# codebydant/sfM_danPipeline

Hardware: AMD Instinct MI355X
Metric: image-pairs matched/sec + BA iterations/sec (200 cams, 100k pts, 1M obs) (higher is better)
Workload: dtype i8

## Files before the change

sfm_danpipeline_amd/csrc/ba.hip:

```cpp
#include "common.h"
#include "ba_front_plan.h"
#include "ba_setup.h"
#include <algorithm>
#include <atomic>
#include <chrono>
#include <cmath>
#include <condition_variable>
#include <cstring>
#include <mutex>
#include <functional>
#include <map>
#include <thread>
#include <vector>
#include <float.h>
#include <unistd.h>

namespace {

constexpr int CAMD = 40;
using bsetup::SC;
constexpr int RED2_SLOTS = 32, RED2_SUM_N = 8 + 4 * RED2_SLOTS, RED2_TMP = RED2_SUM_N, RED2_INFO = RED2_SUM_N + 1,
              RED2_N = RED2_SUM_N + 8;
constexpr int RED2_TIMEOUT = 4;
constexpr int INFO_FINISHER_TIMEOUT = -2;
using bsetup::Chunk;

struct BaDev {
  int nc, np, no, dim, ld;
  const int* optr;
  const int* ocam;
  const double2* oxy;
  double* cams;
  double* pts;
  double* focal;
  double* camd;
  double* cams_c;
  double* pts_c;
  double* focal_c;
  double* camd_c;
  double* scale_c;
  double* scale_p;
  double* iscale_p;
  double* scale_f;
  double* diag;
  double* red;
  double* z;
  double* xinv;
  double* red2;
  int* info;
  struct LmDev* lm;
  double* step_part;
  int step_total;
  int cam_parts;
  int decide_here;
  int rank;
  int step_last;
  double* lm_host;
// ... 395 lines not shown
      asm volatile("s_memtime %0\n\ts_memrealtime %1\n\ts_waitcnt lgkmcnt(0)" : "=s"(t_), "=s"(r_)::"memory"); \
      g_elim_wg[5 * blockIdx.x + slot] = t_;                                                         \
      g_elim_wg[5 * blockIdx.x + 2 + slot] = r_;                                                     \
      if (slot == 0) {                                                                               \
        unsigned id_, xcc_;                                                                          \
        asm volatile("s_getreg_b32 %0, hwreg(HW_REG_HW_ID)\n\ts_getreg_b32 %1, hwreg(HW_REG_XCC_ID)" : "=s"(id_), "=s"(xcc_)); \
        g_elim_wg[5 * blockIdx.x + 4] = ((unsigned long long)xcc_ << 32) | id_;                      \
      }                                                                                              \
    }                                                                                                \
  } while (0)
#define EL_STAMP(slot, cond)                                                         \
  do {                                                                               \
    unsigned long long t_;                                                           \
    asm volatile("s_memtime %0\n\ts_waitcnt lgkmcnt(0)" : "=s"(t_)::"memory");       \
    ((blockIdx.x == 0 && wave == 0 && (cond)) ? g_elim_stamps : g_elim_dump)[slot] = t_; \
  } while (0)
#define EL_STAMPW(slot)                                                        \
  do {                                                                         \
    unsigned long long t_;                                                     \
    asm volatile("s_memtime %0\n\ts_waitcnt lgkmcnt(0)" : "=s"(t_)::"memory"); \
    ((blockIdx.x == 0) ? g_elim_stamps : g_elim_dump)[slot] = t_;              \
  } while (0)
#else
#define EL_STAMP(slot, cond)
#define EL_STAMPW(slot)
#define EL_WG(slot)
#endif
using bsetup::ELIM_SLAB_FF;
using bsetup::ELIM_SLAB;
using bsetup::FP;
constexpr int MP = 80;

typedef __attribute__((address_space(3))) double lds_double;
struct CamLds {
  const lds_double* base;
  const lds_double* dbase;
  __device__ __forceinline__ double operator[](int e) const { return e < 12 ? base[e * 16] : dbase[e * 16]; }
};

#ifndef SFM_ELIM_LB
#define SFM_ELIM_LB __launch_bounds__(512)
#endif
struct ElimShape {
  static constexpr int LP = 10;
  static constexpr int PPW = 64 / LP;
  static constexpr int KST = (3 * PPW + 3) / 4;
  static constexpr int PROWS = 4 * KST;
};
__device__ __forceinline__ void group10_sum12(double (&red)[12], double* R, int lane, int q, int o) {
  constexpr int PR = 66;
  typedef __attribute__((address_space(3))) double ldsd;
  ldsd* Rl = (ldsd*)R;
#pragma unroll
  for (int v = 0; v < 12; ++v) Rl[v * PR + lane] = red[v];
  __builtin_amdgcn_fence(__ATOMIC_RELEASE, "wavefront");
  __builtin_amdgcn_wave_barrier();
  __builtin_amdgcn_fence(__ATOMIC_ACQUIRE, "wavefront");
  const int qq = q < 6 ? q : 5;
  const ldsd* a = Rl + o * PR + qq * 10;
  const ldsd* b = Rl + (10 + (o & 1)) * PR + qq * 10;
  double s0 = a[0], s1 = b[0];
#pragma unroll
  for (int j = 1; j < 10; ++j) {
    s0 += a[j];
    s1 += b[j];
  }
// ... 333 lines not shown
  for (int idx = tid; idx < 36 * FP; idx += (int)blockDim.x) {
    const int e = idx / FP, slot = idx - e * FP;
    if (slot >= n) continue;
    double v = 0.0;
    for (int w = 0; w < nw; ++w) v += s_F[(w * 36 + e) * FP + slot];
    s_F[e * FP + slot] = v;
    if (norms || e >= 33) continue;
    if (e < 21) {
      int i = 0, rem = e;
      while (rem >= 6 - i) {
        rem -= 6 - i;
        ++i;
      }
      g_sub(6 * slot + i, 6 * slot + i + rem, v);
    } else if (e < 27) {
      g_sub(6 * slot + e - 21, 6 * n, v);
    } else {
      g_sub(6 * slot + e - 27, 6 * n + 1, v);
    }
  }
  __syncthreads();
  EL_STAMP(4, true);
  if (tid < 3) {
    double v = 0.0;
    for (int slot = 0; slot < n; ++slot) v += s_F[(33 + tid) * FP + slot];
    s_F[(nw * 36 + tid) * FP] = v;
    if (!norms && tid < 2) g_sub(6 * n, 6 * n + tid, v);
  }
  __syncthreads();
  EL_STAMP(5, true);
  if (slab) {
    double* my = slab + (size_t)chunk_index * ELIM_SLAB;
    if (!norms)
      for (int k = tid; k < NT * 256; k += (int)blockDim.x) my[k] = s_G[k];
    for (int idx = tid; idx < 36 * FP; idx += (int)blockDim.x) my[ELIM_SLAB_FF + idx] = s_F[idx];
    if (tid < 3) my[ELIM_SLAB_FF + 36 * FP + tid] = s_F[(nw * 36 + tid) * FP];
    if (tid == 0) {
      double gm = 0.0, nf = 0.0;
      for (int w = 0; w < nw; ++w) {
        gm = fmax(gm, s_wv[2 * w]);
        nf += s_wv[2 * w + 1];
      }
      my[ELIM_SLAB_FF + 36 * FP + 3] = gm;
      my[ELIM_SLAB_FF + 36 * FP + 4] = nf;
      my[ELIM_SLAB_FF + 36 * FP + 5] = norms ? 0.0 : s_G[g_slot(6 * n, 6 * n)];
      my[ELIM_SLAB_FF + 36 * FP + 6] = norms ? 0.0 : s_G[g_slot(6 * n, 6 * n + 1)];
    }
    EL_STAMP(6, true);
    EL_WG(1);
#ifdef SFM_ELIM_WG_RECORDS
    if (tid == 0 && blockIdx.x < 2048) g_elim_wg[5 * blockIdx.x + 4] |= (unsigned long long)ch.cnt << 48;
#endif
    return;
  }
  double* scv = red_sc(d);
  if (lane == 0 && !norms) {
    if (nfail) atomic_add_f64(scv + 2, (double)nfail);
    atomic_max_pos_f64(scv + SC + rank, gmax);
  }
  for (int idx = tid; idx < 33 * FP; idx += (int)blockDim.x) {
    const int e = idx / FP, slot = idx - e * FP;
    if (slot >= n) continue;
    const int r0 = 6 * cams[slot];
    if (e < 21) {
      int i = 0, rem = e;
      while (rem >= 6 - i) {
        rem -= 6 - i;
        ++i;
      }
      if (rem == 0) atomic_add_f64(red_dc(d) + r0 + i, s_F[e * FP + slot]);
    } else if (e >= 27 && !norms) {
      atomic_add_f64(red_gF(d) + r0 + e - 27, s_F[e * FP + slot]);
    }
  }
  if (tid < 3) {
    const double v = s_F[(nw * 36 + tid) * FP];
    if (tid == 0) atomic_add_f64(red_dc(d) + fo, v);
    else if (norms) {
    } else if (tid == 1) atomic_add_f64(red_gF(d) + fo, v);
// ... 34 lines not shown
    double radius;
    lm_view(d, radius);
    inv_radius = 1.0 / radius;
  }
  elim_chunk<NB>(d, chunks, chunk_ids[blockIdx.x], sig_cams, inv_radius, lm_lo, lm_hi, rank, norms, slab);
}

__global__ __launch_bounds__(256) void ba_gather_slabs(const double* __restrict__ slab, const int* __restrict__ ptr,
                                                       const unsigned* __restrict__ src, const int* __restrict__ dest, int nd,
                                                       double* __restrict__ red, long long gmax_off, const LmDev* __restrict__ lm) {
  if (lm && lm->stop != LM_RUNNING) return;
  const int i = (blockIdx.x * blockDim.x + threadIdx.x) >> 4, j = threadIdx.x & 15;
  const bool live = i < nd;
  const int d = live ? dest[i] : 0;
  const int k0 = live ? ptr[i] : 0, k1 = live ? ptr[i + 1] : 0;
  if (live && d < 0) {
    double v = 0.0;
    for (int k = k0 + j; k < k1; k += 16) v = fmax(v, slab[src[k]]);
#pragma unroll
    for (int off = 8; off > 0; off >>= 1) v = fmax(v, __shfl_xor(v, off, 16));
    if (j == 0) red[gmax_off] = fmax(red[gmax_off], v);
    return;
  }
  double v = 0.0;
  for (int k = k0 + j; k < k1; k += 16) {
    const unsigned sk = src[k];
    const double x = slab[sk & 0x7fffffffu];
    v += (sk >> 31) ? -x : x;
  }
  v = row16_sum(v);
  if (live && j == 0) red[d] += v;
}

__global__ __launch_bounds__(256) void ba_gather_rows(const double* __restrict__ slab,
                                                      const int* __restrict__ colmap, const int4* __restrict__ row_hdr,
                                                      const int4* __restrict__ row_head, const int4* __restrict__ row_src, int nrows,
                                                      int row_wgs, int ld, int accw, int fo, int nchunks, const int* __restrict__ ptr,
                                                      const unsigned* __restrict__ src, const int* __restrict__ dest, int nd,
                                                      double* __restrict__ red, long long gmax_off, int rmw, const LmDev* __restrict__ lm) {
  extern __shared__ double s_acc[];
  if (lm && lm->stop != LM_RUNNING) return;
  if ((int)blockIdx.x == (int)gridDim.x - 1) {
    const int T = blockDim.x, t = threadIdx.x;
    double p[7] = {0, 0, 0, 0, 0, 0, 0};
    for (int c0 = t; c0 < nchunks; c0 += 4 * T) {
      double x[4][7];
#pragma unroll
      for (int u = 0; u < 4; ++u) {
        const double* tail = slab + (size_t)(c0 + u * T < nchunks ? c0 + u * T : c0) * ELIM_SLAB + ELIM_SLAB_FF + 36 * FP;
        x[u][0] = tail[5];
        x[u][1] = tail[6];
#pragma unroll
        for (int q = 0; q < 5; ++q) x[u][2 + q] = tail[q];
      }
      asm volatile("" ::: "memory");
#pragma unroll
      for (int u = 0; u < 4; ++u)
        if (c0 + u * T < nchunks) {
#pragma unroll
          for (int q = 0; q < 7; ++q) p[q] = q == 5 ? fmax(p[q], x[u][q]) : p[q] + x[u][q];
        }
    }
    for (int q = 0; q < 7; ++q) s_acc[q * T + t] = p[q];
    __syncthreads();
    for (int h = T >> 1; h > 0; h >>= 1) {
      if (t < h)
        for (int q = 0; q < 7; ++q) s_acc[q * T + t] = q == 5 ? fmax(s_acc[q * T + t], s_acc[q * T + t + h]) : s_acc[q * T + t] + s_acc[q * T + t + h];
      __syncthreads();
    }
    if (t < 7) {
      const size_t ssz = (size_t)ld * ld;
      const size_t at[7] = {(size_t)fo * ld + fo, ssz + fo, ssz + 2 * (size_t)ld + fo, ssz + (size_t)ld + fo, ssz + 3 * (size_t)ld,
                            (size_t)gmax_off, ssz + 3 * (size_t)ld + 2};
      const double v = s_acc[t * T], o = red[at[t]];
      red[at[t]] = t < 2 ? o - v : t == 5 ? fmax(o, v) : o + v;
    }
    return;
  }
  if ((int)blockIdx.x >= row_wgs) {
    const int i = (((int)blockIdx.x - row_wgs) * blockDim.x + threadIdx.x) >> 4, j = threadIdx.x & 15;
    const bool live = i < nd;
    const int d = live ? dest[i] : 0;
    const int k0 = live ? ptr[i] : 0, k1 = live ? ptr[i + 1] : 0;
    if (live && d < 0) {
      double v = 0.0;
      for (int k = k0 + j; k < k1; k += 16) v = fmax(v, slab[src[k]]);
#pragma unroll
      for (int off = 8; off > 0; off >>= 1) v = fmax(v, __shfl_xor(v, off, 16));
      if (j == 0) red[gmax_off] = fmax(red[gmax_off], v);
      return;
    }
    double v = 0.0;
    for (int k = k0 + j; k < k1; k += 64) {
      unsigned sk[4];
#pragma unroll
      for (int u = 0; u < 4; ++u) sk[u] = k + 16 * u < k1 ? src[k + 16 * u] : 0u;
      double x[4];
#pragma unroll
      for (int u = 0; u < 4; ++u) x[u] = slab[sk[u] & 0x7fffffffu];
#pragma unroll
      for (int u = 0; u < 4; ++u)
        if (k + 16 * u < k1) v += (sk[u] >> 31) ? -x[u] : x[u];
    }
    v = row16_sum(v);
    if (live && j == 0) red[d] += v;
    return;
  }
  const int wave = threadIdx.x >> 6, lane = threadIdx.x & 63, nw = blockDim.x >> 6;
  const int w = blockIdx.x * nw + wave;
  if (w >= nrows) return;
  double* acc = s_acc + (size_t)wave * accw;
  const int4 hdr = row_hdr[w];
  int4 my = lane < 32 ? row_head[(size_t)w * 32 + lane] : make_int4(0, 0, 0, 0);
  const int* const clist = colmap + hdr.w;
  const int nT = 6 * clist[-1], nacc = nT + 4;
  for (int c = lane; c < accw; c += 64) acc[c] = 0.0;
  const int gr = hdr.x, nsrc = hdr.y;
  const int lane_off = (lane >> 4) * 256 + (lane & 15);
  for (int kb = 0; kb < nsrc; kb += 32) {
    constexpr int GB = 32;
    const int m = nsrc - kb < 32 ? nsrc - kb : 32;
    if (kb > 0) my = lane < m ? row_src[hdr.z + (kb - 32) + lane] : make_int4(0, 0, 0, 0);
    for (int u0 = 0; u0 < m; u0 += GB) {
      double v[GB];
      int col[GB];
      bool ok[GB];
#pragma unroll
      for (int u = 0; u < GB; ++u) {
        const int uu = u0 + u < m ? u0 + u : m - 1;
        const int base = __builtin_amdgcn_readlane(my.x, uu), rec = __builtin_amdgcn_readlane(my.y, uu);
        const int cm = __builtin_amdgcn_readlane(my.z, uu), ff = __builtin_amdgcn_readlane(my.w, uu);
        const int lr = rec & 255, n = (rec >> 8) & 255, roff = (int)((unsigned)rec >> 16);
        ok[u] = u0 + u < m && ((lane >= lr && lane < 6 * n + 2) || lane >= 62);
        const int idx = lane >= 62 ? ELIM_SLAB_FF + (lane == 62 ? (ff & 0xFFFF) : (int)((unsigned)ff >> 16)) : roff + lane_off;
        v[u] = slab[(size_t)(unsigned)base + (ok[u] ? idx : 0)];
        col[u] = colmap[cm + lane];
      }
      asm volatile("" ::: "memory");
#pragma unroll
      for (int u = 0; u < GB; ++u)
        if (ok[u]) __hip_atomic_fetch_add((lds_double*)acc + col[u], v[u], __ATOMIC_RELAXED, __HIP_MEMORY_SCOPE_WORKGROUP);
    }
  }
  double* Srow = red + (size_t)gr * ld;
  const size_t ssz = (size_t)ld * ld;
  for (int c = lane; c < nacc; c += 64) {
    const double a = acc[c];
    if (a != 0.0) {
      double* at = c < nT       ? Srow + 6 * clist[c / 6] + c % 6
                   : c == nT     ? Srow + fo
                   : c == nT + 1 ? red + ssz + gr
                   : c == nT + 2 ? red + ssz + 2 * (size_t)ld + gr
                                 : red + ssz + (size_t)ld + gr;
      const double o = rmw ? *at : 0.0;
      *at = c <= nT + 1 ? o - a : o + a;
    }
  }
}

__global__ __launch_bounds__(256) void ba_cam_blocks(BaDev d, const int* __restrict__ cptr,
                                                     const int* __restrict__ cpt,
                                                     const double2* __restrict__ cxy, int nsplit,
                                                     int norms_only ,
                                                     const int2* __restrict__ cslot ,
                                                     const double* __restrict__ T, const double* __restrict__ tfu,
                                                     const double* __restrict__ pp_part, int n_part, int rank,
                                                     double* __restrict__ cb_part ,
                                                     int* __restrict__ cb_cnt ) {
  __shared__ double sh[4][36];
  __shared__ double sh2[4][33];
  __shared__ int s_last;
  {
    double radius_unused;
    lm_view(d, radius_unused);
  }
  double q[33];
#pragma unroll
  for (int e = 0; e < 33; ++e) q[e] = 0.0;
  const int c = blockIdx.x / nsplit, part = blockIdx.x - c * nsplit;
  const int k0 = cptr[c], k1 = cptr[c + 1];
  const int len = k1 - k0;
  const int per = (len + nsplit - 1) / nsplit;
  const int kb = k0 + part * per, ke = min(k1, kb + per);
  double a[36];
#pragma unroll
  for (int e = 0; e < 36; ++e) a[e] = 0.0;
  const double* cd = d.camd + (size_t)CAMD * c;
  const double* scp = norms_only ? nullptr : d.scale_c + 6 * c;
  const double sf = norms_only ? 1.0 : *d.scale_f, focal = *d.focal;
  for (int k = kb + threadIdx.x; k < ke; k += 256) {
// ... 705 lines not shown
        for (int ks = 0; ks < 16; ks += 2) {
          CHOL_MFMA(acc[0], -Lb[0][ks], Lb[0][ks]);
          CHOL_MFMA(acc[1], -Lb[0][ks], Lb[1][ks]);
          CHOL_MFMA(p0, -Lb[0][ks + 1], Lb[0][ks + 1]);
          CHOL_MFMA(p1, -Lb[0][ks + 1], Lb[1][ks + 1]);
        }
        acc[0] += p0;
        acc[1] += p1;
      }
      C2_STAMP(23);
      const double* const y0 = sYb + j16 * CBP + q;
      const double* const y1 = y0 + 16 * CBP;
      int seen = 0;
#pragma unroll 1
      for (int b = 0; b < 8; ++b) {
        if (seen <= b) seen = __builtin_amdgcn_readfirstlane(lds_wait_ge(&s_flag[F_YPROG], b + 1));
        const double Y0 = y0[4 * b], Y1 = y1[4 * b];
        CHOL_MFMA(acc[0], -Y0, Y0);
        CHOL_MFMA(acc[1], -Y0, Y1);
      }
      __builtin_amdgcn_s_setprio(3);
      C2_STAMP(3);
    } else {
      lds_wait_ge(&s_flag[F_CNT_DAA], 3);
      acc[0] = chol2_get(sDa, 0, lane);
      acc[1] = chol2_get(sDa, 2, lane);
      acc[2] = chol2_get(sDa, 3, lane);
    }
    bool bad = false;
    const int c0 = pass ? b0 : a0;
    chol2_potrf_blocks(acc, sAll + opaque(pass * 3 * T), sdi_all + opaque(pass * CB), s_flag + opaque(F_PROG_A + pass),
                       bad, lane, nullptr, ld, pass ? &s_flag[F_DBB_HI] : nullptr);
    C2_STAMP(pass ? 4 : 2);
    if (owner && bad && lane == 0) atomicExch(info, c0 + 1);
    if (!pass) {
      __builtin_amdgcn_s_setprio(1);
      if (pend) {
        double Lb[16];
#pragma unroll
        for (int ks = 0; ks < 16; ++ks) Lb[ks] = opab[32 + 16 + 4 * ks * C2_PAB];
        chol2_fold_regs(t1, Lb, Lb);
      }
      lds_wait_ge(&s_flag[F_YPROG], 8);
      const double* const yh = sYb + (16 + j16) * CBP + q;
      v4d p0 = {0.0, 0.0, 0.0, 0.0}, p1 = p0, p2 = p0;
#pragma unroll
      for (int b = 0; b < 8; b += 4) {
        const double Ya = yh[4 * b], Yb = yh[4 * b + 4], Yc = yh[4 * b + 8], Yd = yh[4 * b + 12];
        CHOL_MFMA(t1, -Ya, Ya);
        CHOL_MFMA(p0, -Yb, Yb);
        CHOL_MFMA(p1, -Yc, Yc);
        CHOL_MFMA(p2, -Yd, Yd);
      }
      t1 += (p0 + p1) + p2;
      chol2_put(sAll + 3 * T, 3, lane, t1);
      lds_flag_add(&s_flag[F_DBB_HI], lane);
      C2_STAMP(14);
    }
    if (!pass && !owner) {
      if (pend) {
        double Lb[16], Lr[2][16];
#pragma unroll
        for (int ks = 0; ks < 16; ++ks) {
          Lb[ks] = opab[32 + 16 + 4 * ks * C2_PAB];
          Lr[0][ks] = oprw[4 * ks * C2_PRW];
          Lr[1][ks] = oprw[16 + 4 * ks * C2_PRW];
        }
// ... 1100 lines not shown

struct sfmhip_ba {
  sfmhip_ctx* ctx = nullptr;
  LmState lm;
  LmDev* d_lm = nullptr;
  LmDev* h_ring = nullptr;
  LmDev* h_ring_dev = nullptr;
  unsigned lm_seq = 0;
  double* d_step_part = nullptr;
  size_t step_part_n = 0;
  bool tree_by_level = false;
  int spin_timeouts = 0;
  int nc = 0, np_in = 0, no_in = 0;
  int np = 0, no = 0;
  int dim = 0, ld = 0;
  size_t ssz = 0;
  BaDev d{};
  bool use_arena = false;
  size_t arena_off = 0, arena_need = 0;
  bool pinned_shared = false;
  std::vector<int> perm;
  std::vector<int> obs_src;
  std::vector<int> cxy_src;
  double2* d_oxy_w = nullptr;
  int* d_obs_src = nullptr;
  std::vector<unsigned char> h_cam_used;
  unsigned char* d_cam_used = nullptr;
  bool cam_used_known = false;
  double* d_flag = nullptr;
  bool chol_attr_set = false;
  Chunk* d_chunks = nullptr;
  bool elim_deterministic = !(getenv("SFMHIP_BA_DETERMINISTIC") && atoi(getenv("SFMHIP_BA_DETERMINISTIC")) == 0);
  double* d_slab = nullptr;
  int* d_gth_ptr[2] = {nullptr, nullptr};
  unsigned* d_gth_src[2] = {nullptr, nullptr};
  int* d_gth_dest[2] = {nullptr, nullptr};
  int n_gth[2] = {0, 0};
  int4* d_grow_hdr = nullptr;
  int4* d_grow_head = nullptr;
  int4* d_grow_src = nullptr;
  int* d_grow_colmap = nullptr;
  int n_grow = 0, grow_waves = 4, grow_accw = 64, n_chunks = 0;
  int* d_chunk_ids[8] = {nullptr, nullptr, nullptr, nullptr, nullptr, nullptr, nullptr, nullptr};
  int n_chunk_ids[8] = {0, 0, 0, 0, 0, 0, 0, 0};
  int* d_sig_cams = nullptr;
  int* d_cptr = nullptr;
  int* d_cpt = nullptr;
  double2* d_cxy = nullptr;
  int cam_split = 1;
  int dense_xb = 0;
  double* d_back_part = nullptr;
  double* d_cb_part = nullptr;
  int* d_cb_cnt = nullptr;
  int* d_fb_points = nullptr;
  int* d_pp_obase = nullptr;
  int n_fb = 0;
  int2* d_cslot = nullptr;
  double* d_ppT = nullptr;
  double* d_tfu = nullptr;
  double* d_pp_part = nullptr;
  int n_pp_part = 0;
  int* d_pair_ptr = nullptr;
  int2* d_pair_cams = nullptr;
  int2* d_pair_ent = nullptr;
  int n_pairs_pp = 0;
  long long tree_dbg_ints = 0, tree_dbg_doubles = 0;
// ... 249 lines not shown
  double2* d_oxy = nullptr;
  b->red_count = b->ssz + 3 * (size_t)b->ld + SC + 64 + RED2_N + b->ssz;
#define BA_A(ptr, n)                         \
  if (rc == SFMHIP_OK) rc = ba_alloc(b, &(ptr), (size_t)(n))
  BA_A(d_optr, b->np + 1);
  BA_A(d_ocam, b->no);
  BA_A(d_oxy, b->no);
  BA_A(b->d_obs_src, b->no);
  BA_A(d.cams, 6 * n_cam);
  BA_A(d.pts, 3 * (size_t)b->np);
  BA_A(d.focal, 1);
  BA_A(d.camd, (size_t)CAMD * n_cam);
  BA_A(d.cams_c, 6 * n_cam);
  BA_A(d.pts_c, 3 * (size_t)b->np);
  BA_A(d.focal_c, 1);
  BA_A(d.camd_c, (size_t)CAMD * n_cam);
  BA_A(d.scale_c, 6 * n_cam);
  BA_A(d.scale_p, 3 * (size_t)b->np);
  BA_A(d.iscale_p, 3 * (size_t)b->np);
  BA_A(d.scale_f, 1);
  BA_A(d.diag, b->ld);
  BA_A(d.red, b->red_count);
  BA_A(d.z, b->ld);
  if (rc == SFMHIP_OK) {
    d.red2 = d.red + b->ssz + 3 * (size_t)b->ld + SC + 64;
    d.info = (int*)(d.red2 + RED2_INFO);
    d.xinv = d.red2 + RED2_N;
  }
  BA_A(b->d_cam_used, n_cam);
  BA_A(b->d_flag, 2);
  BA_A(b->d_chunks, S.chunks.size());
  if (!S.gth_dest[0].empty() || !S.gth_dest[1].empty() || !S.grow_hdr.empty()) {
    BA_A(b->d_slab, S.chunks.size() * (size_t)ELIM_SLAB);
    for (int m = 0; m < 2; ++m) {
      BA_A(b->d_gth_ptr[m], S.gth_ptr[m].size());
      BA_A(b->d_gth_src[m], S.gth_src[m].size());
      BA_A(b->d_gth_dest[m], S.gth_dest[m].size());
    }
    if (!S.grow_hdr.empty()) {
      BA_A(b->d_grow_hdr, S.grow_hdr.size());
      BA_A(b->d_grow_head, S.grow_head.size());
      BA_A(b->d_grow_src, S.grow_over.size());
      BA_A(b->d_grow_colmap, S.grow_colmap.size());
    }
  }
  for (int c = 0; c < 8; ++c) BA_A(b->d_chunk_ids[c], S.ids[c].size());
  BA_A(b->d_sig_cams, S.sig_cams.size());
  BA_A(b->d_cptr, S.cptr.size());
  BA_A(b->d_cpt, S.cpt.size());
  BA_A(b->d_cxy, S.cpt.size());
  BA_A(b->d_fb_points, S.fb.size());
  BA_A(b->d_pp_obase, S.pp_obase.size());
  BA_A(b->d_cslot, S.cslot.size());
  BA_A(b->d_ppT, 18 * S.cslot.size());
  BA_A(b->d_tfu, 6 * S.fb.size());
  b->n_pp_part = (int)((S.fb.size() * PP_LANES + 255) / 256);
  BA_A(b->d_pp_part, 8 * (size_t)b->n_pp_part);
  if (b->cam_split > 1) {
    BA_A(b->d_cb_part, 66 * (size_t)n_cam * b->cam_split);
    BA_A(b->d_cb_cnt, n_cam);
    if (rc == SFMHIP_OK && hipMemset(b->d_cb_cnt, 0, sizeof(int) * (size_t)n_cam) != hipSuccess) rc = SFMHIP_ERR_HIP;
  }
  {
    const int nt = b->ld / CB;
    b->dense_xb = nt >= DENSE_XB_MIN_NT ? DENSE_XB : 0;
    if (b->dense_xb) {
// ... 3 lines not shown
  }
  BA_A(b->d_pair_ptr, S.pair_ptr.size());
  BA_A(b->d_pair_cams, S.pair_cams.size());
  BA_A(b->d_pair_ent, S.pair_ent.size());
#undef BA_A
  if (rc != SFMHIP_OK) return rc;
  d.optr = d_optr;
  d.ocam = d_ocam;
  d.oxy = d_oxy;
  b->d_oxy_w = d_oxy;
  for (int c = 0; c < 8; ++c) b->n_chunk_ids[c] = (int)S.ids[c].size();
  b->n_fb = (int)S.fb.size();
  auto up = [&](void* dst, const void* src, size_t bytes) -> hipError_t {
    return bytes ? hipMemcpy(dst, src, bytes, hipMemcpyHostToDevice) : hipSuccess;
  };
  lap_("hipMalloc x27");
  SFM_HIP_TRY(up(d_optr, S.optr.data(), S.optr.size() * 4));
  SFM_HIP_TRY(up(d_ocam, S.ocam.data(), S.ocam.size() * 4));
  SFM_HIP_TRY(up(b->d_obs_src, b->obs_src.data(), b->obs_src.size() * 4));
  SFM_TRY(ba_upload_xy(b, obs_xy, n_obs));
  SFM_HIP_TRY(up(b->d_cam_used, b->h_cam_used.data(), n_cam));
  SFM_HIP_TRY(up(b->d_chunks, S.chunks.data(), S.chunks.size() * sizeof(Chunk)));
  b->n_chunks = (int)S.chunks.size();
  if (!S.bs_desc.empty()) {
    SFM_TRY(ba_alloc(b, &b->d_bs_ids, S.bs_desc.size()));
    SFM_HIP_TRY(hipMemcpy(b->d_bs_ids, S.bs_desc.data(), S.bs_desc.size() * sizeof(int), hipMemcpyHostToDevice));
  }
  for (int m = 0; m < 2 && b->d_slab; ++m) {
    SFM_HIP_TRY(up(b->d_gth_ptr[m], S.gth_ptr[m].data(), S.gth_ptr[m].size() * 4));
    SFM_HIP_TRY(up(b->d_gth_src[m], S.gth_src[m].data(), S.gth_src[m].size() * 4));
    SFM_HIP_TRY(up(b->d_gth_dest[m], S.gth_dest[m].data(), S.gth_dest[m].size() * 4));
    b->n_gth[m] = (int)S.gth_dest[m].size();
  }
  if (b->d_slab && !S.grow_hdr.empty()) {
    SFM_HIP_TRY(up(b->d_grow_hdr, S.grow_hdr.data(), S.grow_hdr.size() * sizeof(int4)));
    SFM_HIP_TRY(up(b->d_grow_head, S.grow_head.data(), S.grow_head.size() * sizeof(int4)));
    SFM_HIP_TRY(up(b->d_grow_src, S.grow_over.data(), S.grow_over.size() * sizeof(int4)));
    SFM_HIP_TRY(up(b->d_grow_colmap, S.grow_colmap.data(), S.grow_colmap.size() * 4));
    b->n_grow = (int)S.grow_hdr.size();
  }
  for (int c = 0; c < 8; ++c) SFM_HIP_TRY(up(b->d_chunk_ids[c], S.ids[c].data(), S.ids[c].size() * 4));
  SFM_HIP_TRY(up(b->d_sig_cams, S.sig_cams.data(), S.sig_cams.size() * 4));
  SFM_HIP_TRY(up(b->d_cptr, S.cptr.data(), S.cptr.size() * 4));
  SFM_HIP_TRY(up(b->d_cpt, S.cpt.data(), S.cpt.size() * 4));
  SFM_HIP_TRY(up(b->d_cxy, S.cxy.data(), S.cxy.size() * 8));
  SFM_HIP_TRY(up(b->d_fb_points, S.fb.data(), S.fb.size() * 4));
  SFM_HIP_TRY(up(b->d_pp_obase, S.pp_obase.data(), S.pp_obase.size() * 4));
  SFM_HIP_TRY(up(b->d_cslot, S.cslot.data(), S.cslot.size() * sizeof(int2)));
  SFM_HIP_TRY(up(b->d_pair_ptr, S.pair_ptr.data(), S.pair_ptr.size() * 4));
  SFM_HIP_TRY(up(b->d_pair_cams, S.pair_cams.data(), S.pair_cams.size() * sizeof(int2)));
  SFM_HIP_TRY(up(b->d_pair_ent, S.pair_ent.data(), S.pair_ent.size() * sizeof(int2)));
  b->n_pairs_pp = (int)S.pair_cams.size();
  lap_("uploads");
  const size_t sc_bytes = (sizeof(double) * (SC + 64 + RED2_N + 1) + 255) & ~(size_t)255, ring_bytes = sizeof(LmDev) * LM_RING;
  if (arena) {
    if (ctx->ba_pinned_bytes < sc_bytes + ring_bytes) {
      if (ctx->ba_pinned) hipHostFree(ctx->ba_pinned);
      ctx->ba_pinned = nullptr, ctx->ba_pinned_bytes = 0;
      SFM_HIP_TRY(hipHostMalloc(&ctx->ba_pinned, sc_bytes + ring_bytes, hipHostMallocDefault));
      ctx->ba_pinned_bytes = sc_bytes + ring_bytes;
    }
    b->pinned_shared = true;
    b->h_sc = (double*)ctx->ba_pinned;
    b->h_ring = (LmDev*)((char*)ctx->ba_pinned + sc_bytes);
  } else {
    SFM_HIP_TRY(hipHostMalloc((void**)&b->h_sc, sizeof(double) * (SC + 64 + RED2_N + 1), hipHostMallocDefault));
// ... 160 lines not shown
    if (i < dim) {
      const size_t at = (size_t)i * ld + dim - 1;
      if (unpack) redw[at] = packed[base + i];
      else packed[base + i] = red[at];
    } else {
      if (unpack) redw[ssz + i - dim] = packed[base + i];
      else packed[base + i] = red[ssz + i - dim];
    }
  }
}

static int ba_allreduce(sfmhip_ba* b, double* buf, size_t count) {
  if (b->world <= 1) return SFMHIP_OK;
  const int rc = b->allreduce(buf, count, b->allreduce_user);
  return rc == 0 ? SFMHIP_OK : SFMHIP_ERR_COMM;
}

static int ba_agree_flag(sfmhip_ba* b, int* flag) {
  hipStream_t st = b->ctx->stream;
  double* slot = b->d_flag;
  double v = *flag ? 1.0 : 0.0;
  SFM_HIP_TRY(hipMemcpyAsync(slot, &v, sizeof(double), hipMemcpyHostToDevice, st));
  SFM_TRY(ba_allreduce(b, slot, 1));
  SFM_HIP_TRY(hipMemcpyAsync(&v, slot, sizeof(double), hipMemcpyDeviceToHost, st));
  SFM_HIP_TRY(hipStreamSynchronize(st));
  *flag = v > 0.5 ? 1 : 0;
  return SFMHIP_OK;
}

static int ba_launch_eliminate(sfmhip_ba* b, double inv_radius, double lm_lo, double lm_hi, int norms) {
  hipStream_t st = b->ctx->stream;
  int nl = 0;
  double* slab = b->elim_deterministic ? b->d_slab : nullptr;
#define BA_ELIM(NB)                                                                                                   \
  for (int cls = 0; cls < 2; ++cls) {                                                                                 \
    const int li = 4 * cls + NB - 1, nthreads = cls ? 64 : 256;                                                       \
    if (!b->n_chunk_ids[li]) continue;                                                                                \
                                 \
    const size_t nw_ = nthreads / 64, gram_ = (size_t)(NB * (NB + 1) / 2) * 256;                                      \
                                          \
    const size_t red_ = nw_ == 4 ? (size_t)4 * std::min(NB * (NB + 1) / 2, 5) * 256 : 0;                              \
    const size_t prows_ = ElimShape::PROWS;                                                                           \
    const size_t lds = sizeof(double) * (nw_ * 36 * FP + 3 * FP + std::max(std::max(nw_ * prows_ * MP, gram_), red_)); \
    hipLaunchKernelGGL((ba_eliminate_mfma<NB>), dim3(b->n_chunk_ids[li]), dim3(nthreads), lds, st, b->d,              \
                       b->d_chunks, b->d_chunk_ids[li],                                                               \
                       b->d_sig_cams, inv_radius, lm_lo, lm_hi, b->rank, norms, slab);                                \
    ++nl;                                                                                                             \
  }
  BA_ELIM(1)
  BA_ELIM(2)
  BA_ELIM(3)
  BA_ELIM(4)
#undef BA_ELIM
  const int m = norms ? 1 : 0;
  if (slab && nl && m == 0 && b->n_grow) {
    const int rw = (b->n_grow + b->grow_waves - 1) / b->grow_waves, gw = (b->n_gth[0] * 16 + 64 * b->grow_waves - 1) / (64 * b->grow_waves);
    const size_t lds_g = sizeof(double) * std::max((size_t)b->grow_accw * b->grow_waves, (size_t)7 * 64 * b->grow_waves);
    hipLaunchKernelGGL(ba_gather_rows, dim3(rw + gw + 1), dim3(64 * b->grow_waves), lds_g, st,
                       (const double*)slab, (const int*)b->d_grow_colmap, (const int4*)b->d_grow_hdr,
                       (const int4*)b->d_grow_head, (const int4*)b->d_grow_src, b->n_grow, rw, b->ld, b->grow_accw, 6 * b->nc, b->n_chunks, (const int*)b->d_gth_ptr[0],
                       (const unsigned*)b->d_gth_src[0], (const int*)b->d_gth_dest[0], b->n_gth[0], b->d.red,
                       (long long)(b->ssz + 3 * (size_t)b->ld + SC + b->rank), b->n_fb ? 1 : 0, (const LmDev*)b->d.lm);
    ++nl;
  } else if (slab && nl && b->n_gth[m]) {
    hipLaunchKernelGGL(ba_gather_slabs, dim3((b->n_gth[m] + 15) / 16), dim3(256), 0, st, (const double*)slab,
                       (const int*)b->d_gth_ptr[m], (const unsigned*)b->d_gth_src[m], (const int*)b->d_gth_dest[m], b->n_gth[m],
// ... 863 lines not shown
  }
  SFM_TRY(ba_step_eval(b, b->lm.s.radius, o));
  if (b->ctx->timing) {
    SFM_HIP_TRY(hipEventRecord(b->ev[4], st));
    b->ev_on[4] = true;
  }
  return SFMHIP_OK;
}

static int ba_wait_record(sfmhip_ba* b, unsigned seq, LmDev* out) {
  volatile LmDev* slot = b->h_ring + seq % LM_RING;
  const auto t0 = std::chrono::steady_clock::now();
  unsigned spins = 0;
  while (slot->seq != seq) {
    if ((++spins & 0xFFF) == 0 && std::chrono::duration<double>(std::chrono::steady_clock::now() - t0).count() > 0.02) {
      SFM_HIP_TRY(hipStreamSynchronize(b->ctx->stream));
      if (slot->seq != seq) return SFMHIP_ERR_HIP;
      break;
    }
  }
  std::atomic_thread_fence(std::memory_order_acquire);
  memcpy(out, (const void*)slot, sizeof(LmDev));
  return SFMHIP_OK;
}

static int ba_handle_timeout(sfmhip_ba* b, int info) {
  b->spin_timeouts += 1;
  {
    const std::vector<unsigned long long> pend(b->step_part_n, STEP_PENDING);
    SFM_HIP_TRY(hipMemcpyAsync(b->d_step_part, pend.data(), sizeof(double) * b->step_part_n, hipMemcpyHostToDevice, b->ctx->stream));
    SFM_HIP_TRY(hipStreamSynchronize(b->ctx->stream));
  }
  if (info == INFO_FINISHER_TIMEOUT) return SFMHIP_ERR_TIMEOUT;
  if (b->tree_on && !b->tree_by_level) {
    b->tree_by_level = true;
    return SFMHIP_OK;
  }
  return SFMHIP_ERR_TIMEOUT;
}

static int ba_lm_loop(sfmhip_ba* b, const sfmhip_ba_opts* o, int iters, const std::function<double()>& elapsed, int* term) {
  const bool t_only = iters >= 0;
  hipStream_t st = b->ctx->stream;
  LmDev& s = b->lm.s;
  lm_set_options(s, o, t_only);
  *term = SFMHIP_BA_NO_CONVERGENCE;
  const char* hl = getenv("SFMHIP_BA_HOST_LOOP");
  const bool host_loop = (hl && atoi(hl) != 0) || b->ctx->timing;
  if (!t_only) {
    if (s.iter >= s.max_iter) return SFMHIP_OK;
    if (s.radius < s.min_radius) {
      *term = SFMHIP_BA_CONVERGENCE;
      return SFMHIP_OK;
    }
  }
  auto time_is_up = [&](int* up) -> int {
    *up = 0;
    if (t_only || !(o->max_time_s > 0)) return SFMHIP_OK;
    *up = elapsed() >= o->max_time_s ? 1 : 0;
    if (b->world > 1) SFM_TRY(ba_agree_flag(b, up));
    return SFMHIP_OK;
  };
  int done = 0;
  if (host_loop) {
    b->d.lm = nullptr;
    s.seq = b->lm_seq;
// ... 472 lines not shown
```

sfm_danpipeline_amd/csrc/ba_front.h:

```cpp
#pragma once

#define FR_MFMA_SUB(acc, a, b) acc = __builtin_amdgcn_mfma_f64_16x16x4f64(a, b, acc, 0, 0, 1)

#ifdef SFM_FRONT_STAMPS
__device__ unsigned long long g_front_stamps[128][128];
#define FR_STAMP(slot)                                                            \
  do {                                                                            \
    unsigned long long t_;                                                        \
    asm volatile("s_memtime %0\n\ts_waitcnt lgkmcnt(0)" : "=s"(t_)::"memory");    \
    if (f < 128 && lane == 0) g_front_stamps[f][slot] = t_;                       \
  } while (0)
#define FR_STAMP_REAL(slot)                                                       \
  do {                                                                            \
    unsigned long long t_;                                                        \
    asm volatile("s_memrealtime %0\n\ts_waitcnt lgkmcnt(0)" : "=s"(t_)::"memory"); \
    if (f < 128 && lane == 0) g_front_stamps[f][slot] = t_;                       \
  } while (0)
__device__ unsigned long long g_down_stamps[128][8];
#define FD_STAMP(slot)                                                            \
  do {                                                                            \
    unsigned long long t_;                                                        \
    asm volatile("s_memrealtime %0\n\ts_waitcnt lgkmcnt(0)" : "=s"(t_)::"memory"); \
    if (f < 128 && threadIdx.x == 0) g_down_stamps[f][slot] = t_;                 \
  } while (0)
// ... 551 lines not shown
    __builtin_amdgcn_s_setprio(3);
    v4d dacc[3] = {t[0][0], t[0][1], t[0][3]};
    bool bad = false;
#pragma unroll 1
    for (int j = 0; j < no; ++j) {
      const int gen = j & 1, base = 8 * (j >> 1), nbj = opaque_s(j == no - 1 ? D.nb_last : 8);
      if (j >= 2) lds_wait_ge(s_flag + FRC_CONS + gen, FR_WAVES * (j >> 1));
      FR_STAMP(4 + 3 * j);
      fr_potrf(dacc, sD + gen * FR_TILE, sdi + gen * CB, progL_of(gen), base, nbj, bad, lane, pool_rs, (D.offL + (CB * j) * ldk + CB * j) * 8, ldk);
      FR_STAMP(5 + 3 * j);
      if (j + 1 < no) {
        lds_wait_ge(s_flag + FRC_DREADY, j + 1);
        dacc[0] = chol2_get(sDg, 0, lane);
        dacc[1] = chol2_get(sDg, 2, lane);
        dacc[2] = chol2_get(sDg, 3, lane);
        lds_flag_set(s_flag + FRC_DTAKEN, j + 1);
        const double* const y0 = panel_tile(gen, j + 1) + (lane & 15) * CBP + (lane >> 4);
        const int* const pr = prog_of(gen, j + 1);
        int seen = 0;
#pragma unroll
        for (int kb = 0; kb < 8; ++kb) {
          if (kb < nbj) {
            if (seen < base + kb + 1) seen = __builtin_amdgcn_readfirstlane(lds_wait_ge(pr, base + kb + 1));
            const double Y0 = y0[4 * kb], Y1 = y0[16 * CBP + 4 * kb];
            FR_MFMA_SUB(dacc[0], Y0, Y0);
            FR_MFMA_SUB(dacc[1], Y0, Y1);
            FR_MFMA_SUB(dacc[2], Y1, Y1);
          }
        }
      }
      FR_STAMP(6 + 3 * j);
      lds_flag_add(s_flag + FRC_CONS + gen, lane);
    }
    if (bad && lane == 0) atomicExch(d.info, 1 + sInv[0]);
  } else if (rhs) {
#pragma unroll 1
    for (int j = 0; j < no; ++j) {
      const int gen = j & 1, base = 8 * (j >> 1), nbj = opaque_s(j == no - 1 ? D.nb_last : 8);
      if (j >= 2) lds_wait_ge(s_flag + FRC_CONS + gen, FR_WAVES * (j >> 1));
      const double* const sL = sD + gen * FR_TILE;
      const double* const sdj = sdi + gen * CB;
      double* const yj = sy + CB * j;
      const int col = lane & 31;
      double yv = yj[col];
#pragma unroll
      for (int b = 0; b < 8; ++b) {
        if (b < nbj) {
          const int c = 4 * b;
          lds_wait_ge(progL_of(gen), base + b + 1);
          const double y0 = readlane_f64(yv, c), y1 = readlane_f64(yv, c + 1), y2 = readlane_f64(yv, c + 2), y3 = readlane_f64(yv, c + 3);
          const double l10 = sL[(c + 1) * CBP + c];
          const v2d l2 = *(const v2d*)(sL + (c + 2) * CBP + c);
          const v2d l3 = *(const v2d*)(sL + (c + 3) * CBP + c);
          const double l32 = sL[(c + 3) * CBP + c + 2];
          const v2d r01 = *(const v2d*)(sdj + c), r23 = *(const v2d*)(sdj + c + 2);
          const double x0 = y0 * r01.x;
          const double x1 = (y1 - x0 * l10) * r01.y;
          const double x2 = (y2 - x0 * l2.x - x1 * l2.y) * r23.x;
          const double x3 = (y3 - x0 * l3.x - x1 * l3.y - x2 * l32) * r23.y;
          const v2d la = *(const v2d*)(sL + col * CBP + c), lb = *(const v2d*)(sL + col * CBP + c + 2);
          if (col > c + 3) yv -= la.x * x0 + la.y * x1 + lb.x * x2 + lb.y * x3;
          yv = col == c ? x0 : col == c + 1 ? x1 : col == c + 2 ? x2 : col == c + 3 ? x3 : yv;
        }
      }
      if (lane < CB) yj[lane] = yv;
      asm volatile("" ::: "memory");
      const int h = lane >> 5, kn = 4 * nbj;
// ... 525 lines not shown
```

Measured before the change: 1.895 million.

## Fuse Schur elimination and row gather into one kernel with per-chunk flags

After: 1.896 million, median of 3. No clear change (+0.0%).

```diff
diff --git a/sfm_danpipeline_amd/csrc/ba.hip b/sfm_danpipeline_amd/csrc/ba.hip
--- a/sfm_danpipeline_amd/csrc/ba.hip
+++ b/sfm_danpipeline_amd/csrc/ba.hip
@@ -23,6 +23,7 @@
               RED2_N = RED2_SUM_N + 8;
 constexpr int RED2_TIMEOUT = 4;
 constexpr int INFO_FINISHER_TIMEOUT = -2;
+constexpr int INFO_GATHER_TIMEOUT = -3;
 using bsetup::Chunk;
 
 struct BaDev {
@@ -484,6 +485,13 @@
 constexpr int MP = 80;
 
 typedef __attribute__((address_space(3))) double lds_double;
+typedef __attribute__((address_space(1))) double slab_gbl_double;
+__device__ __forceinline__ void slab_st(double* p, double v) {
+  __hip_atomic_store((slab_gbl_double*)p, v, __ATOMIC_RELAXED, __HIP_MEMORY_SCOPE_AGENT);
+}
+__device__ __forceinline__ double slab_ld(const double* p) {
+  return __hip_atomic_load((const slab_gbl_double*)p, __ATOMIC_RELAXED, __HIP_MEMORY_SCOPE_AGENT);
+}
 struct CamLds {
   const lds_double* base;
   const lds_double* dbase;
@@ -883,19 +891,19 @@
   if (slab) {
     double* my = slab + (size_t)chunk_index * ELIM_SLAB;
     if (!norms)
-      for (int k = tid; k < NT * 256; k += (int)blockDim.x) my[k] = s_G[k];
-    for (int idx = tid; idx < 36 * FP; idx += (int)blockDim.x) my[ELIM_SLAB_FF + idx] = s_F[idx];
-    if (tid < 3) my[ELIM_SLAB_FF + 36 * FP + tid] = s_F[(nw * 36 + tid) * FP];
+      for (int k = tid; k < NT * 256; k += (int)blockDim.x) slab_st(my + k, s_G[k]);
+    for (int idx = tid; idx < 36 * FP; idx += (int)blockDim.x) slab_st(my + ELIM_SLAB_FF + idx, s_F[idx]);
+    if (tid < 3) slab_st(my + ELIM_SLAB_FF + 36 * FP + tid, s_F[(nw * 36 + tid) * FP]);
     if (tid == 0) {
       double gm = 0.0, nf = 0.0;
       for (int w = 0; w < nw; ++w) {
         gm = fmax(gm, s_wv[2 * w]);
         nf += s_wv[2 * w + 1];
       }
-      my[ELIM_SLAB_FF + 36 * FP + 3] = gm;
-      my[ELIM_SLAB_FF + 36 * FP + 4] = nf;
-      my[ELIM_SLAB_FF + 36 * FP + 5] = norms ? 0.0 : s_G[g_slot(6 * n, 6 * n)];
-      my[ELIM_SLAB_FF + 36 * FP + 6] = norms ? 0.0 : s_G[g_slot(6 * n, 6 * n + 1)];
+      slab_st(my + ELIM_SLAB_FF + 36 * FP + 3, gm);
+      slab_st(my + ELIM_SLAB_FF + 36 * FP + 4, nf);
+      slab_st(my + ELIM_SLAB_FF + 36 * FP + 5, norms ? 0.0 : s_G[g_slot(6 * n, 6 * n)]);
+      slab_st(my + ELIM_SLAB_FF + 36 * FP + 6, norms ? 0.0 : s_G[g_slot(6 * n, 6 * n + 1)]);
     }
     EL_STAMP(6, true);
     EL_WG(1);
@@ -996,26 +1004,41 @@
   if (live && j == 0) red[d] += v;
 }
 
-__global__ __launch_bounds__(256) void ba_gather_rows(const double* __restrict__ slab,
-                                                      const int* __restrict__ colmap, const int4* __restrict__ row_hdr,
-                                                      const int4* __restrict__ row_head, const int4* __restrict__ row_src, int nrows,
-                                                      int row_wgs, int ld, int accw, int fo, int nchunks, const int* __restrict__ ptr,
-                                                      const unsigned* __restrict__ src, const int* __restrict__ dest, int nd,
-                                                      double* __restrict__ red, long long gmax_off, int rmw, const LmDev* __restrict__ lm) {
+typedef __attribute__((address_space(1))) unsigned slab_gbl_u32;
+__device__ __forceinline__ int slab_poll(const unsigned* flag, unsigned epoch) {
+  int budget = 1 << 17;
+  while (__hip_atomic_load((const slab_gbl_u32*)flag, __ATOMIC_RELAXED, __HIP_MEMORY_SCOPE_AGENT) != epoch) {
+    if (--budget == 0) return 1;
+    __builtin_amdgcn_s_sleep(2);
+  }
+  return 0;
+}
+template <int GB , bool VSRC>
+__device__ __forceinline__ void gather_rows_wg(int blk, int nblk, const unsigned* __restrict__ flags, unsigned epoch, int* __restrict__ info,
+                                               const double* __restrict__ slab,
+                                               const int* __restrict__ colmap, const int4* __restrict__ row_hdr,
+                                               const int4* __restrict__ row_head, const int4* __restrict__ row_src, int nrows,
+                                               int row_wgs, int ld, int accw, int fo, int nchunks, const int* __restrict__ ptr,
+                                               const unsigned* __restrict__ src, const int* __restrict__ dest, int nd,
+                                               double* __restrict__ red, long long gmax_off, int rmw) {
   extern __shared__ double s_acc[];
-  if (lm && lm->stop != LM_RUNNING) return;
-  if ((int)blockIdx.x == (int)gridDim.x - 1) {
+  if (blk == nblk - 1) {
     const int T = blockDim.x, t = threadIdx.x;
     double p[7] = {0, 0, 0, 0, 0, 0, 0};
+    int to = 0;
     for (int c0 = t; c0 < nchunks; c0 += 4 * T) {
+      if (flags)
+        for (int u = 0; u < 4; ++u)
+          if (c0 + u * T < nchunks && !to) to = slab_poll(flags + c0 + u * T, epoch);
+      asm volatile("" ::: "memory");
       double x[4][7];
 #pragma unroll
       for (int u = 0; u < 4; ++u) {
         const double* tail = slab + (size_t)(c0 + u * T < nchunks ? c0 + u * T : c0) * ELIM_SLAB + ELIM_SLAB_FF + 36 * FP;
-        x[u][0] = tail[5];
-        x[u][1] = tail[6];
-#pragma unroll
-        for (int q = 0; q < 5; ++q) x[u][2 + q] = tail[q];
+        x[u][0] = slab_ld(tail + 5);
+        x[u][1] = slab_ld(tail + 6);
+#pragma unroll
+        for (int q = 0; q < 5; ++q) x[u][2 + q] = slab_ld(tail + q);
       }
       asm volatile("" ::: "memory");
 #pragma unroll
@@ -1025,6 +1048,7 @@
           for (int q = 0; q < 7; ++q) p[q] = q == 5 ? fmax(p[q], x[u][q]) : p[q] + x[u][q];
         }
     }
+    if (to) atomicMin(info, INFO_GATHER_TIMEOUT);
     for (int q = 0; q < 7; ++q) s_acc[q * T + t] = p[q];
     __syncthreads();
     for (int h = T >> 1; h > 0; h >>= 1) {
@@ -1041,8 +1065,8 @@
     }
     return;
   }
-  if ((int)blockIdx.x >= row_wgs) {
-    const int i = (((int)blockIdx.x - row_wgs) * blockDim.x + threadIdx.x) >> 4, j = threadIdx.x & 15;
+  if (blk >= row_wgs) {
+    const int i = ((blk - row_wgs) * blockDim.x + threadIdx.x) >> 4, j = threadIdx.x & 15;
     const bool live = i < nd;
     const int d = live ? dest[i] : 0;
     const int k0 = live ? ptr[i] : 0, k1 = live ? ptr[i + 1] : 0;
@@ -1071,7 +1095,7 @@
     return;
   }
   const int wave = threadIdx.x >> 6, lane = threadIdx.x & 63, nw = blockDim.x >> 6;
-  const int w = blockIdx.x * nw + wave;
+  const int w = blk * nw + wave;
   if (w >= nrows) return;
   double* acc = s_acc + (size_t)wave * accw;
   const int4 hdr = row_hdr[w];
@@ -1082,28 +1106,33 @@
   const int gr = hdr.x, nsrc = hdr.y;
   const int lane_off = (lane >> 4) * 256 + (lane & 15);
   for (int kb = 0; kb < nsrc; kb += 32) {
-    constexpr int GB = 32;
     const int m = nsrc - kb < 32 ? nsrc - kb : 32;
     if (kb > 0) my = lane < m ? row_src[hdr.z + (kb - 32) + lane] : make_int4(0, 0, 0, 0);
+    if (flags) {
+      if (lane < m && slab_poll(flags + (unsigned)my.x / (unsigned)ELIM_SLAB, epoch)) atomicMin(info, INFO_GATHER_TIMEOUT);
+      asm volatile("" ::: "memory");
+    }
     for (int u0 = 0; u0 < m; u0 += GB) {
       double v[GB];
       int col[GB];
       bool ok[GB];
+      int okv[GB];
 #pragma unroll
       for (int u = 0; u < GB; ++u) {
         const int uu = u0 + u < m ? u0 + u : m - 1;
-        const int base = __builtin_amdgcn_readlane(my.x, uu), rec = __builtin_amdgcn_readlane(my.y, uu);
-        const int cm = __builtin_amdgcn_readlane(my.z, uu), ff = __builtin_amdgcn_readlane(my.w, uu);
+        const int base = VSRC ? __shfl(my.x, uu) : __builtin_amdgcn_readlane(my.x, uu), rec = VSRC ? __shfl(my.y, uu) : __builtin_amdgcn_readlane(my.y, uu);
+        const int cm = VSRC ? __shfl(my.z, uu) : __builtin_amdgcn_readlane(my.z, uu), ff = VSRC ? __shfl(my.w, uu) : __builtin_amdgcn_readlane(my.w, uu);
         const int lr = rec & 255, n = (rec >> 8) & 255, roff = (int)((unsigned)rec >> 16);
         ok[u] = u0 + u < m && ((lane >= lr && lane < 6 * n + 2) || lane >= 62);
+        if (VSRC) okv[u] = __builtin_amdgcn_readfirstlane(0) + (ok[u] ? 1 : 0);
         const int idx = lane >= 62 ? ELIM_SLAB_FF + (lane == 62 ? (ff & 0xFFFF) : (int)((unsigned)ff >> 16)) : roff + lane_off;
-        v[u] = slab[(size_t)(unsigned)base + (ok[u] ? idx : 0)];
+        v[u] = slab_ld(slab + (size_t)(unsigned)base + (ok[u] ? idx : 0));
         col[u] = colmap[cm + lane];
       }
       asm volatile("" ::: "memory");
 #pragma unroll
       for (int u = 0; u < GB; ++u)
-        if (ok[u]) __hip_atomic_fetch_add((lds_double*)acc + col[u], v[u], __ATOMIC_RELAXED, __HIP_MEMORY_SCOPE_WORKGROUP);
+        if (VSRC ? okv[u] != 0 : ok[u]) __hip_atomic_fetch_add((lds_double*)acc + col[u], v[u], __ATOMIC_RELAXED, __HIP_MEMORY_SCOPE_WORKGROUP);
     }
   }
   double* Srow = red + (size_t)gr * ld;
@@ -1120,6 +1149,49 @@
       *at = c <= nT + 1 ? o - a : o + a;
     }
   }
+}
+
+__global__ __launch_bounds__(256) void ba_gather_rows(const double* __restrict__ slab,
+                                                      const int* __restrict__ colmap, const int4* __restrict__ row_hdr,
+                                                      const int4* __restrict__ row_head, const int4* __restrict__ row_src, int nrows,
+                                                      int row_wgs, int ld, int accw, int fo, int nchunks, const int* __restrict__ ptr,
+                                                      const unsigned* __restrict__ src, const int* __restrict__ dest, int nd,
+                                                      double* __restrict__ red, long long gmax_off, int rmw, const LmDev* __restrict__ lm) {
+  if (lm && lm->stop != LM_RUNNING) return;
+  gather_rows_wg<32, false>((int)blockIdx.x, (int)gridDim.x, nullptr, 0u, nullptr, slab, colmap, row_hdr, row_head, row_src, nrows, row_wgs, ld, accw, fo,
+                 nchunks, ptr, src, dest, nd, red, gmax_off, rmw);
+}
+
+struct GatherArgs {
+  const int* colmap;
+  const int4 *row_hdr, *row_head, *row_src;
+  int nrows, row_wgs, ld, accw, fo, nchunks;
+  long long gmax_off;
+  int rmw;
+};
+template <int NB>
+__global__ SFM_ELIM_LB void ba_elim_gather(BaDev d, const Chunk* __restrict__ chunks, const int* __restrict__ chunk_ids, int n_elim,
+                                           const int* __restrict__ sig_cams, double inv_radius, double lm_lo, double lm_hi, int rank,
+                                           int norms ,
+                                           double* __restrict__ slab, unsigned* __restrict__ flags, unsigned epoch,
+                                           const GatherArgs* __restrict__ gp) {
+  if (lm_stopped(d)) return;
+  if ((int)blockIdx.x < n_elim) {
+    if (d.lm) {
+      double radius;
+      lm_view(d, radius);
+      inv_radius = 1.0 / radius;
+    }
+    elim_chunk<NB>(d, chunks, chunk_ids[blockIdx.x], sig_cams, inv_radius, lm_lo, lm_hi, rank, norms, slab);
+    asm volatile("s_waitcnt vmcnt(0)" ::: "memory");
+    __syncthreads();
+    if (threadIdx.x == 0)
+      __hip_atomic_store((slab_gbl_u32*)(flags + chunk_ids[blockIdx.x]), epoch, __ATOMIC_RELAXED, __HIP_MEMORY_SCOPE_AGENT);
+    return;
+  }
+  const GatherArgs g = *gp;
+  gather_rows_wg<8, false>((int)blockIdx.x - n_elim, (int)gridDim.x - n_elim, flags, epoch, d.info, slab, g.colmap, g.row_hdr, g.row_head, g.row_src,
+                 g.nrows, g.row_wgs, g.ld, g.accw, g.fo, g.nchunks, nullptr, nullptr, nullptr, 0, d.red, g.gmax_off, g.rmw);
 }
 
 __global__ __launch_bounds__(256) void ba_cam_blocks(BaDev d, const int* __restrict__ cptr,
@@ -1891,7 +1963,7 @@
     chol2_potrf_blocks(acc, sAll + opaque(pass * 3 * T), sdi_all + opaque(pass * CB), s_flag + opaque(F_PROG_A + pass),
                        bad, lane, nullptr, ld, pass ? &s_flag[F_DBB_HI] : nullptr);
     C2_STAMP(pass ? 4 : 2);
-    if (owner && bad && lane == 0) atomicExch(info, c0 + 1);
+    if (owner && bad && lane == 0) atomicCAS(info, 0, c0 + 1);
     if (!pass) {
       __builtin_amdgcn_s_setprio(1);
       if (pend) {
@@ -3058,6 +3130,11 @@
   Chunk* d_chunks = nullptr;
   bool elim_deterministic = !(getenv("SFMHIP_BA_DETERMINISTIC") && atoi(getenv("SFMHIP_BA_DETERMINISTIC")) == 0);
   double* d_slab = nullptr;
+  unsigned* d_slab_flag = nullptr;
+  unsigned slab_epoch = 0;
+  GatherArgs* d_fuse_args = nullptr;
+  int fuse_args_rw = -1;
+  bool fuse_gather = !(getenv("SFMHIP_BA_FUSE") && atoi(getenv("SFMHIP_BA_FUSE")) == 0);
   int* d_gth_ptr[2] = {nullptr, nullptr};
   unsigned* d_gth_src[2] = {nullptr, nullptr};
   int* d_gth_dest[2] = {nullptr, nullptr};
@@ -3373,6 +3450,8 @@
   BA_A(b->d_chunks, S.chunks.size());
   if (!S.gth_dest[0].empty() || !S.gth_dest[1].empty() || !S.grow_hdr.empty()) {
     BA_A(b->d_slab, S.chunks.size() * (size_t)ELIM_SLAB);
+    BA_A(b->d_slab_flag, S.chunks.size());
+    BA_A(b->d_fuse_args, 1);
     for (int m = 0; m < 2; ++m) {
       BA_A(b->d_gth_ptr[m], S.gth_ptr[m].size());
       BA_A(b->d_gth_src[m], S.gth_src[m].size());
@@ -3442,6 +3521,8 @@
     SFM_HIP_TRY(up(b->d_gth_dest[m], S.gth_dest[m].data(), S.gth_dest[m].size() * 4));
     b->n_gth[m] = (int)S.gth_dest[m].size();
   }
+  if (b->d_slab_flag) SFM_HIP_TRY(hipMemset(b->d_slab_flag, 0, S.chunks.size() * sizeof(unsigned)));
+  b->fuse_args_rw = -1;
   if (b->d_slab && !S.grow_hdr.empty()) {
     SFM_HIP_TRY(up(b->d_grow_hdr, S.grow_hdr.data(), S.grow_hdr.size() * sizeof(int4)));
     SFM_HIP_TRY(up(b->d_grow_head, S.grow_head.data(), S.grow_head.size() * sizeof(int4)));
@@ -3668,6 +3749,40 @@
   hipStream_t st = b->ctx->stream;
   int nl = 0;
   double* slab = b->elim_deterministic ? b->d_slab : nullptr;
+  if (slab && !norms && b->n_grow && b->fuse_gather && b->d_slab_flag && b->n_gth[0] == 0) {
+    int only = -1, nonempty = 0;
+    for (int li = 0; li < 8; ++li)
+      if (b->n_chunk_ids[li]) ++nonempty, only = li;
+    if (nonempty == 1 && b->n_chunk_ids[only] == b->n_chunks) {
+      const int cls = only / 4, NB = only % 4 + 1, nthreads = cls ? 64 : 256;
+      const size_t nw_ = nthreads / 64, gram_ = (size_t)(NB * (NB + 1) / 2) * 256;
+      const size_t red_ = nw_ == 4 ? (size_t)4 * std::min(NB * (NB + 1) / 2, 5) * 256 : 0;
+      const size_t lds = sizeof(double) * (nw_ * 36 * FP + 3 * FP + std::max(std::max(nw_ * (size_t)ElimShape::PROWS * MP, gram_), red_));
+      const size_t lds_g = sizeof(double) * std::max((size_t)b->grow_accw * nw_, (size_t)7 * nthreads);
+      if (lds_g <= lds) {
+        const int rw = (int)((b->n_grow + nw_ - 1) / nw_), ne = b->n_chunk_ids[only];
+        const unsigned epoch = ++b->slab_epoch;
+        if (b->fuse_args_rw != rw) {
+          const GatherArgs g{(const int*)b->d_grow_colmap, (const int4*)b->d_grow_hdr,
+                             (const int4*)b->d_grow_head, (const int4*)b->d_grow_src, b->n_grow, rw, b->ld, b->grow_accw, 6 * b->nc,
+                             b->n_chunks, (long long)(b->ssz + 3 * (size_t)b->ld + SC + b->rank), b->n_fb ? 1 : 0};
+          SFM_HIP_TRY(hipMemcpyAsync(b->d_fuse_args, &g, sizeof(GatherArgs), hipMemcpyHostToDevice, st));
+          SFM_HIP_TRY(hipStreamSynchronize(st));
+          b->fuse_args_rw = rw;
+        }
+#define BA_ELIM_GATHER(NBV)                                                                                                  \
+  if (NB == NBV)                                                                                                            \
+    hipLaunchKernelGGL((ba_elim_gather<NBV>), dim3(ne + rw + 1), dim3(nthreads), lds, st, b->d, b->d_chunks, b->d_chunk_ids[only], ne, \
+                       b->d_sig_cams, inv_radius, lm_lo, lm_hi, b->rank, 0, slab, b->d_slab_flag, epoch, b->d_fuse_args);
+        BA_ELIM_GATHER(1)
+        BA_ELIM_GATHER(2)
+        BA_ELIM_GATHER(3)
+        BA_ELIM_GATHER(4)
+#undef BA_ELIM_GATHER
+        return 1;
+      }
+    }
+  }
 #define BA_ELIM(NB)                                                                                                   \
   for (int cls = 0; cls < 2; ++cls) {                                                                                 \
     const int li = 4 * cls + NB - 1, nthreads = cls ? 64 : 256;                                                       \
@@ -4597,6 +4712,10 @@
     SFM_HIP_TRY(hipStreamSynchronize(b->ctx->stream));
   }
   if (info == INFO_FINISHER_TIMEOUT) return SFMHIP_ERR_TIMEOUT;
+  if (info == INFO_GATHER_TIMEOUT && b->fuse_gather) {
+    b->fuse_gather = false;
+    return SFMHIP_OK;
+  }
   if (b->tree_on && !b->tree_by_level) {
     b->tree_by_level = true;
     return SFMHIP_OK;
diff --git a/sfm_danpipeline_amd/csrc/ba_front.h b/sfm_danpipeline_amd/csrc/ba_front.h
--- a/sfm_danpipeline_amd/csrc/ba_front.h
+++ b/sfm_danpipeline_amd/csrc/ba_front.h
@@ -607,7 +607,7 @@
       FR_STAMP(6 + 3 * j);
       lds_flag_add(s_flag + FRC_CONS + gen, lane);
     }
-    if (bad && lane == 0) atomicExch(d.info, 1 + sInv[0]);
+    if (bad && lane == 0) atomicCAS(d.info, 0, 1 + sInv[0]);
   } else if (rhs) {
 #pragma unroll 1
     for (int j = 0; j < no; ++j) {
```
